# thomasjoergensen/RFAnalyzer

Measured on AMD Instinct MI355X. Metric: IQ Msamples/s + waterfall lines/s at 64k FFT; achieved HBM GB/s vs roofline, higher is better.
Workload: dtype f32; 1 GPU; config3: 65536-pt FFT, blackman window, s8 IQ, EMA + peak-hold, ring 500 rows, one stream per GPU; fft_size=65536, frames_per_call=500, input_format=s8, parallelism=streams1, avg=ema, ring_rows=500

## Files before the change

rfanalyzer_amd/csrc/engine.hip:

```cpp
#include <hip/hip_runtime.h>

#include <algorithm>
#include <cmath>
#include <cstdio>
#include <cstdlib>
#include <cstring>
#include <new>
#include <string>
#include <vector>

#include "../../include/rfa.h"
#include "fft_kernels.h"
#include "framer.h"

static constexpr size_t kStampWords = (size_t)2048 * 16 * 8;

using rfa::FftLaunch;

struct WinPlan {
    int count = 0;
    int block_bins = 0, n_jobs = 0, n_pieces = 0, n_folds = 0, n_slots = 0;
    void *d_plan = nullptr;
    size_t d_plan_cap = 0;
    float *d_out = nullptr;
// ... 893 lines not shown
    if (h->chan_on && h->have_tuning) {
        const float samples_per_hz = (float)n / (float)h->last_sample_rate;
        const int64_t f0 = h->last_frequency - h->last_sample_rate / 2;
        auto idx = [&](int64_t f) {
            const float x = (float)(f - f0) * samples_per_hz;
            const long long i = std::isnan(x) ? 0 : x >= 2147483647.0f ? 2147483647LL : x <= -2147483648.0f ? -2147483648LL
                                                                                                               : (long long)x;
            return (int)std::min<long long>(std::max<long long>(i, 0), n);
        };
        chan_first = idx(h->chan_start);
        chan_last = idx(h->chan_end);
    }
    const bool need_chan = chan_last > chan_first;
    h->chan_count = 0;
    h->chan_offset = 0;
    const bool need_win = h->win.count > 0;
    h->win.frames = h->win.offset = 0;
    float *state_rows = rows;
    bool rows_in_ring = false;
    if ((need_state || need_chan || need_win) && !rows) {
        if (h->d_ring && n_frames <= (size_t)h->ring_rows) {
            rows_in_ring = true;
        } else {
            int rc = ensure_device_buffer(h, (void **)&h->d_rows, &h->d_rows_cap, n_frames * (size_t)n * sizeof(float));
            if (rc) return rc;
            state_rows = h->d_rows;
        }
    }
    const bool flip = (long long)n_frames == (long long)h->ring_rows;
    const bool pipe = h->pipe_cus > 0 && need_state && rows_in_ring &&
                      (flip || (long long)n_frames + h->pipe_prev_frames <= (long long)h->ring_rows);
    if (!pipe) {
        int rc = join(h);
        if (rc) return rc;
    }
    const int par = (int)(h->pipe_k & 1);
    hipStream_t fft_stream = h->stream, state_stream = h->stream;
    if (pipe) {
        fft_stream = h->pipe_fft[h->logn > 17 ? 0 : par];
        state_stream = h->pipe_state;
        HIPCHK(h, hipEventRecord(h->pipe_in, h->stream));
        HIPCHK(h, hipStreamWaitEvent(fft_stream, h->pipe_in, 0));
        if (h->pipe_recorded[par]) HIPCHK(h, hipStreamWaitEvent(fft_stream, h->pipe_state_done[par], 0));
        if (flip) {
            std::swap(h->d_ring, h->d_ring_tmp);
            h->generation++;
        }
    }
    const bool raise_ok = h->d_peaks_st && h->d_state_part && rows_in_ring && !pipe &&
                          h->logn == 16 && (fmt == RFA_IN_S8 || fmt == RFA_IN_U8) && window == h->d_window &&
                          h->variant != 1 && h->diag == 0 && !h->d_stamps && (h->ring_logrs & rfa::kRingTile) &&
                          h->stage && (((uintptr_t)in | (uintptr_t)stride) & 15) == 0 &&
                          rfa::state_fused_plan(n, (int)n_frames, h->state_chunks, h->state_fused, nullptr, nullptr);
    const bool raise = raise_ok && h->shadow_fresh;
    FftLaunch a;
    a.in = (const uint8_t *)in;
    a.frame_stride = (long long)stride;
    a.n_frames = (int)n_frames;
    a.fmt = fmt;
    a.window = window;
    a.rows = state_rows;
    if (raise) a.peaks_st = h->d_peaks_st;
    if (pipe) a.cus = h->pipe_fft_cus;
    if (h->d_ring) {
        a.ring = h->d_ring;
        a.ring_rows = h->ring_rows;
        a.ring_base = h->write_index;
        a.ring_first = (int)std::max<long long>(0, (long long)n_frames - h->ring_rows);
        a.ring_logrs = h->ring_logrs;
    }
    int rc = launch_main(h, a, fft_stream);
    if (rc) return rc;
    if (pipe) {
        HIPCHK(h, hipEventRecord(h->pipe_fft_done[par], fft_stream));
        HIPCHK(h, hipStreamWaitEvent(state_stream, h->pipe_fft_done[par], 0));
    }
    if (need_state || need_chan || need_win) {
        rfa::StateLaunch s;
        s.n = n;
        s.n_frames = (int)n_frames;
        s.peaks = h->d_peaks;
        s.ema = h->d_ema;
        s.ema_alpha = h->cfg.ema_alpha;
        s.part = h->d_state_part;
        s.max_chunks = h->state_chunks;
        s.fused = h->state_fused;
        s.first_frame = (int)std::max<long long>(0, (long long)n_frames - rfa::ema_tail_frames(h->cfg.ema_alpha));
        s.peaks_st = raise_ok ? h->d_peaks_st : nullptr;
        s.raised = raise;
        s.stream = state_stream;
        if (rows_in_ring) {
            s.rows = h->d_ring;
            s.ring_rows = h->ring_rows;
            s.ring_base = h->write_index;
            s.ring_logrs = h->ring_logrs;
        } else {
            s.rows = state_rows;
            s.row_stride = n;
        }
        if (need_state) HIPCHK(h, rfa::launch_state(s));
        if (h->d_peaks) h->shadow_fresh = raise_ok;
        if (need_chan) {
            const int spans = rfa::channel_mean_spans(chan_last - chan_first);
            const size_t words = n_frames * (size_t)(spans > 1 ? 1 + spans : 1);
            if (pipe && words * sizeof(float) > h->d_chan_cap)
                HIPCHK(h, hipStreamSynchronize(state_stream));
            int rc = ensure_device_buffer(h, (void **)&h->d_chan, &h->d_chan_cap, words * sizeof(float));
            if (rc) return rc;
            HIPCHK(h, rfa::launch_channel_mean(s, chan_first, chan_last, h->d_chan,
                                               spans > 1 ? h->d_chan + n_frames : nullptr));
            h->chan_count = n_frames;
        }
        if (need_win) {
            rfa::WinLaunch w;
            w.rows = s.rows;
            w.row_stride = s.row_stride;
            w.ring_rows = s.ring_rows;
            w.ring_base = s.ring_base;
            w.ring_dir = -1;
            w.ring_logrs = s.ring_logrs;
            w.n_frames = (int)n_frames;
            w.stream = state_stream;
            int rc = run_windows(h, h->win, w, pipe ? state_stream : nullptr);
            if (rc) return rc;
        }
    }
    if (pipe) {
        HIPCHK(h, hipEventRecord(h->pipe_state_done[par], state_stream));
        h->pipe_recorded[par] = true;
        h->pipe_pending = true;
        h->pipe_prev_frames = (int)n_frames;
        h->pipe_k++;
    }
    if (h->d_ring) {
        const long long R = h->ring_rows;
        const long long last = (long long)n_frames - 1;
        for (long long f = std::max<long long>(0, (long long)n_frames - R); f < (long long)n_frames; f++)
            h->dirty[(size_t)((((long long)h->write_index - f) % R + R) % R)] = 1;
        h->read_index = (int)((((long long)h->write_index - last) % R + R) % R);
        h->write_index = h->read_index == 0 ? h->ring_rows - 1 : h->read_index - 1;
// ... 588 lines not shown
```

rfanalyzer_amd/csrc/fft_kernels.h:

```cpp
#pragma once

#include <hip/hip_runtime.h>
#include <stdint.h>

#include <vector>

namespace rfa {

constexpr int kRingTile = 0x100;
__host__ __device__ __forceinline__ int ring_lr(int code) { return code & 0xff; }
__host__ __device__ __forceinline__ int ring_logm(int code, int logn) { return logn - (code & 0xff); }
__host__ __device__ __forceinline__ int tile_pos(int i) {
    return (((i >> 6) & 15) << 11) | ((i >> 12) << 8) | ((i & 63) << 2) | ((i >> 10) & 3);
}
__host__ __device__ __forceinline__ int tile_sub(int p) {
    return ((((p >> 8) & 7) << 2 | (p & 3)) << 10) | ((p >> 11) << 6) | ((p >> 2) & 63);
}
constexpr int kRingTile2 = 0x200;
__host__ __device__ __forceinline__ int tile2_pos(int i) {
    const int k0 = i & 31, k1 = (i >> 5) & 31, tp = i >> 10;
    return ((k0 >> 1) << 11) | ((tp >> 2) << 8) | (((k0 & 1) | (k1 << 1)) << 2) | (tp & 3);
}
__host__ __device__ __forceinline__ int tile2_sub(int p) {
    const int w = p >> 11, j = (p >> 8) & 7, l = (p >> 2) & 63, e = p & 3;
    return ((l & 1) | (w << 1)) | ((l >> 1) << 5) | ((4 * j + e) << 10);
}
__host__ __device__ __forceinline__ int ring_pos(int t, int code, int logm) {
    const int lr = code & 0xff, sub = t >> lr;
    return ((t & ((1 << lr) - 1)) << logm) |
           ((code & kRingTile) ? tile_pos(sub) : (code & kRingTile2) ? tile2_pos(sub) : sub);
}
__host__ __device__ __forceinline__ int ring_bin(int p, int code, int logm) {
    const int lr = code & 0xff, q = p & ((1 << logm) - 1);
    return (((code & kRingTile) ? tile_sub(q) : (code & kRingTile2) ? tile2_sub(q) : q) << lr) | (p >> logm);
}

constexpr int kMaxLogM = 14;
constexpr int kMaxLogSplit = 3;

struct FftLaunch {
    const uint8_t *in = nullptr;
    long long frame_stride = 0;
    int n_frames = 0;
    int fmt = 0;
    int logn = 0;
    const float *window = nullptr;
    const float *window_il = nullptr;
    const float4 *window_cw = nullptr;
    const float2 *wide_tw = nullptr;
    const float2 *w64_tw = nullptr;
    const float2 *tw_coarse = nullptr;
    const float2 *tw_fine = nullptr;
    int tw_shift = 0;
    float *rows = nullptr;
    float *ring = nullptr;
    int ring_rows = 0;
    int ring_base = 0;
    int ring_first = 0;
    int ring_logrs = 0;
    float2 *complex_out = nullptr;
    float *peaks_st = nullptr;
    int dif_ss = 0;
    int stage = 1;
    int variant = 0;
    int diag = 0;
    unsigned long long *stamps = nullptr;
    int prio = 0;
    int phase_ticks = 0;
    int cus = 0;
    hipStream_t stream = nullptr;
};

hipError_t launch_fft(const FftLaunch &a);
bool wide_supported(int logn);
int ring_logrs_for(int logn, int fmt);
bool w64_format(int fmt);
constexpr int kWidePT = 32;
#ifndef RFA_RES16K
#define RFA_RES16K 0
#endif
inline int wide_logm(int logn) { return logn <= 14 ? logn : (RFA_RES16K && logn == 16 ? 14 : 15); }
std::vector<float2> wide_twiddles(int logn, int pt, int lm);
hipError_t launch_fft_wide(const FftLaunch &a);
std::vector<float2> w64_twiddles();
hipError_t launch_fft64(const FftLaunch &a);

struct DifLaunch {
    const uint8_t *in = nullptr;
    long long frame_stride = 0;
    int n_frames = 0;
    int fmt = 0;
    int logn = 0;
    const float *window = nullptr;
    const float2 *tw_c = nullptr;
    const float2 *tw_d = nullptr;
    const float2 *tw_cp = nullptr;
    const float2 *tw_dp = nullptr;
    float2 *z = nullptr;
    int pipe = 6;
    hipStream_t stream = nullptr;
};
constexpr int kDitLogM = 15;
constexpr int kMaxLogN = 20;
constexpr int kFmtDif = 5;
hipError_t launch_dif_front(const DifLaunch &a);
hipError_t launch_cols_to_rows(const float *cols, float *rows, int n_frames, int logn, hipStream_t st);
int dif_lo_points(bool pipe);
void dif_twiddles(int logn, int lo, std::vector<float2> &c, std::vector<float2> &d);

struct StateLaunch {
    const float *rows = nullptr;
    long long row_stride = 0;
    int ring_rows = 0;
    int ring_base = 0;
    int ring_logrs = 0;
    int n_frames = 0;
    int n = 0;
    float *peaks = nullptr;
    float *ema = nullptr;
    float ema_alpha = 0.f;
    float4 *part = nullptr;
    int max_chunks = 1;
    int fused = 1;
    int first_frame = 0;
    float *peaks_st = nullptr;
    bool raised = false;
    hipStream_t stream = nullptr;
};
hipError_t launch_state(const StateLaunch &a);
int ema_tail_frames(float alpha);
bool state_fused_plan(int n, int n_frames, int max_chunks, int fused, int *chunks, int *chunk_len);
int channel_mean_spans(int width);
hipError_t launch_channel_mean(const StateLaunch &a, int first, int last, float *out, float *partial);

struct DrawLaunch {
    const float *ring = nullptr;
    const float *peaks = nullptr;
    int ring_rows = 0, n = 0, read_index = 0;
    int ring_logrs = 0;
    int width = 0, fft_height = 0, avg_length = 0;
    int start = 0, first_pixel = 0, last_pixel = 0;
    float samples_per_px = 0.f, min_db = 0.f, db_width = 0.f, scale = 0.f;
    const unsigned *colormap = nullptr;
    int colormap_size = 0;
    unsigned *colors = nullptr;
    const int2 *rows = nullptr;
    int n_rows = 0;
    float *avg_rows = nullptr;
    float *path_y = nullptr;
    float *peaks_y = nullptr;
    float *autoscale = nullptr;
    hipStream_t stream = nullptr;
};
hipError_t launch_draw(const DrawLaunch &a);
hipError_t launch_row_windows(const float *row, int ring_logrs, int n, const int *lo, const int *hi, int count,
                              float *peak, float *avg, hipStream_t s);

struct WinLaunch {
    const float *rows = nullptr;
    long long row_stride = 0;
    int ring_rows = 0, ring_base = 0, ring_dir = -1;
    int ring_logrs = 0;
    int n = 0, n_frames = 0;
    int n_windows = 0;
    int block_bins = 0;
    const int4 *jobs = nullptr;
    int n_jobs = 0;
    const int4 *pieces = nullptr;
    const int4 *folds = nullptr;
    int n_folds = 0, n_slots = 0;
    float *peak = nullptr, *avg = nullptr;
    double *psum = nullptr;
    float *pmax = nullptr;
    hipStream_t stream = nullptr;
};
constexpr int kWinNarrow = 32;
constexpr int kWinWave = 1024;
inline int win_piece_bins(int n) { return n < 4096 ? n : 4096; }
inline int win_block_bins(int n, int ring_code) {
    return (ring_code & (kRingTile | kRingTile2)) ? 4096 << ring_lr(ring_code) : win_piece_bins(n);
}
hipError_t launch_batch_windows(const WinLaunch &a);

hipError_t launch_fill(float *p, long long count, float value, hipStream_t s);
// ... 12 lines not shown
```

rfanalyzer_amd/csrc/fft_kernels.hip:

```cpp
#include <hip/hip_runtime.h>
#include <math.h>

#include <algorithm>
#include <cstdlib>
#include <type_traits>

#include "fft_common.h"
#include "fft_kernels.h"
#include "wave.h"

namespace rfa {
template <int LOGM>
struct Geo {
    static constexpr int M = 1 << LOGM;
    static constexpr int TPF = M / 16;
    static constexpr int SLOTS = TPF >= 256 ? 1 : 256 / TPF;
    static constexpr int THREADS = TPF * SLOTS;
    static constexpr int PADM = M + M / 8;
    static constexpr int NP16 = LOGM / 4;
    static constexpr int LASTR = 1 << (LOGM % 4);
    static constexpr int NPASS = NP16 + (LASTR > 1 ? 1 : 0);
};

__device__ __forceinline__ int pad(int e) { return e + ((e >> 4) << 1); }
// ... 439 lines not shown
        const float4 x4 = *reinterpret_cast<const float4 *>(state_row(a, f) + bin);
        const float xs[4] = {x4.x, x4.y, x4.z, x4.w};
#pragma unroll
        for (int k = 0; k < 4; k++) state_step(pk[k], nan[k], emi[k], b[k], xs[k], al);
        am *= keep;
    }
    float4 *out = a.part + (size_t)c * a.n + bin;
#pragma unroll
    for (int k = 0; k < 4; k++) out[k] = state_summary(pk[k], nan[k], am, b[k], emi[k]);
}

__global__ void state_combine_kernel(StateLaunch a, int chunks) {
    const int pos = blockIdx.x * blockDim.x + threadIdx.x;
    if (pos >= a.n) return;
    const int lr = state_logrs(a), bin = ring_bin(pos, lr, ring_logm(lr, ilog2_dev(a.n)));
    float pk = a.peaks ? a.peaks[bin] : 0.f;
    float em = a.ema ? a.ema[bin] : 0.f;
    for (int c = 0; c < chunks; c++) {
        const float4 p = a.part[(size_t)c * a.n + pos];
        pk = peak_max(pk, p.x);
        em = (!state_finite(em) || p.y < 0.0f) ? p.w : fmaf(p.y, em, p.z);
    }
    if (a.peaks) a.peaks[bin] = pk;
    if (a.ema) a.ema[bin] = em;
}

#ifndef RFA_STATE_BUF
#define RFA_STATE_BUF 1
#endif
#ifndef RFA_STATE_UNROLL
#define RFA_STATE_UNROLL 4
#endif
#ifndef RFA_STATE_LOAD_AUX
#define RFA_STATE_LOAD_AUX 0
#endif
template <int CH, bool RAISED = false>
__global__ void __launch_bounds__(256) state_fused_kernel(StateLaunch a, int chunk_len) {
    constexpr int TPC = 256 / CH, BPB = 4 * TPC;
    __shared__ float4 part[CH][BPB];
    const int c = threadIdx.x / TPC, l = threadIdx.x % TPC;
    const int bin = blockIdx.x * BPB + 4 * l;
    const int tail = a.n_frames - a.first_frame;
    {
        const int f0 = a.first_frame + c * chunk_len, f1 = min(a.n_frames, f0 + chunk_len);
        const float al = a.ema_alpha, keep = 1.0f - al;
        float pk[4], emi[4], b[4];
        bool nan[4];
#pragma unroll
        for (int k = 0; k < 4; k++) pk[k] = emi[k] = -INFINITY, b[k] = 0.0f, nan[k] = false;
        float am = 1.0f;
        auto step = [&](float4 x4) {
            const float xs[4] = {x4.x, x4.y, x4.z, x4.w};
#pragma unroll
            for (int k = 0; k < 4; k++) {
                if constexpr (RAISED) {
                    emi[k] = ema_step(emi[k], xs[k], al);
                    b[k] = fmaf(al, xs[k] - b[k], b[k]);
                } else {
                    state_step(pk[k], nan[k], emi[k], b[k], xs[k], al);
                }
            }
            am *= keep;
        };
        auto peak_step = [&](float4 x4) {
            const float xs[4] = {x4.x, x4.y, x4.z, x4.w};
#pragma unroll
            for (int k = 0; k < 4; k++) pk[k] = fmaxf(pk[k], xs[k]), nan[k] |= xs[k] != xs[k];
        };
        auto frames = [&](int fa, int fb, auto &&each) {
            if (RFA_STATE_BUF && a.ring_rows > 0 && (long long)a.ring_rows * a.n * 4 < (1ll << 31)) {
                const unsigned rowb = (unsigned)a.n * 4u;
                const rsrc_t rs = make_rsrc(a.rows, (unsigned)a.ring_rows * rowb);
                int rr = (a.ring_base - fa) % a.ring_rows;
                if (rr < 0) rr += a.ring_rows;
#pragma unroll RFA_STATE_UNROLL
                for (int f = fa; f < fb; f++) {
                    each(__builtin_bit_cast(float4, __builtin_amdgcn_raw_buffer_load_b128(rs, (int)((unsigned)rr * rowb + (unsigned)bin * 4u), 0, RFA_STATE_LOAD_AUX)));
                    rr = rr == 0 ? a.ring_rows - 1 : rr - 1;
                }
            } else {
#pragma unroll 4
                for (int f = fa; f < fb; f++) each(*reinterpret_cast<const float4 *>(state_row(a, f) + bin));
            }
        };
        if constexpr (!RAISED) {
            if (a.first_frame > 0 && a.peaks) {
                const int plen = (a.first_frame + CH - 1) / CH;
                frames(min(a.first_frame, c * plen), min(a.first_frame, (c + 1) * plen), peak_step);
            }
        }
        frames(f0, f1, step);
#pragma unroll
        for (int k = 0; k < 4; k++) part[c][4 * l + k] = state_summary(pk[k], nan[k], am, b[k], emi[k]);
    }
    __syncthreads();
    const int lr = state_logrs(a), lm = ring_logm(lr, ilog2_dev(a.n));
    const bool full = (CH - 1) * chunk_len < tail;
    for (int i = threadIdx.x; i < BPB; i += 256) {
        const int pos = blockIdx.x * BPB + i, gb = ring_bin(pos, lr, lm);
        float p = a.peaks ? a.peaks[gb] : 0.f;
        float em = a.ema ? a.ema[gb] : 0.f;
        if constexpr (RAISED) p = peak_max(p, a.peaks_st[pos]);
        auto fold = [&](auto all) {
#pragma unroll
            for (int cc = 0; cc < CH; cc++) {
                const bool any = decltype(all)::value || cc * chunk_len < tail;
                const float4 q = part[cc][i];
                if constexpr (!RAISED) p = peak_max(p, q.x);
                em = !any ? em : (!state_finite(em) || q.y < 0.0f) ? q.w : fmaf(q.y, em, q.z);
            }
        };
        if (full) fold(std::true_type{});
        else fold(std::false_type{});
        if (a.peaks) a.peaks[gb] = p;
        if (a.peaks && a.peaks_st) a.peaks_st[pos] = p;
        if (a.ema) a.ema[gb] = em;
    }
}

#ifdef RFA_AB_BUILD
static const bool kStateTileOff = std::getenv("RFA_STATE_TILE") && std::atoi(std::getenv("RFA_STATE_TILE")) == 0;
#else
static constexpr bool kStateTileOff = false;
#endif

bool state_fused_plan(int n, int n_frames, int max_chunks, int fused, int *chunks, int *chunk_len) {
    const int c = std::min(max_chunks, (n_frames + 7) / 8);
    if (c < 8 || !fused) return false;
    const int ch = c >= 32 ? 32 : c >= 16 ? 16 : 8;
    if (n % (1024 / ch)) return false;
    if (chunks) *chunks = ch;
    if (chunk_len) *chunk_len = (n_frames + ch - 1) / ch;
    return true;
}

int ema_tail_frames(float alpha) {
    const double keep = 1.0 - (double)alpha, bound = std::ldexp(1.0, -51);
    if (!(keep > 0.0)) return 1;
    if (!(keep < 1.0)) return 0x7fffffff;
    const double t0 = std::ceil(std::log(bound) / std::log(keep));
    if (!(t0 < 1.0e9)) return 0x7fffffff;
    int t = std::max(1, (int)t0);
    while (t > 1 && std::pow(keep, t - 1) <= bound) t--;
    while (std::pow(keep, t) > bound) t++;
    return t;
}

hipError_t launch_state(const StateLaunch &a) {
    if (a.n_frames <= 0) return hipSuccess;
    const int tpb = 256;
    if (a.raised && !(a.peaks && a.peaks_st && state_fused_plan(a.n, a.n_frames, a.max_chunks, a.fused, nullptr, nullptr) &&
                      a.part && (a.ring_logrs & kRingTile)))
        return hipErrorInvalidValue;
    if (a.ring_rows > 0 && !(a.ring_logrs & kRingTile) && a.ring_logrs >= 3 && a.ring_logrs <= 5 && !kStateTileOff) {
        const int m = a.n >> a.ring_logrs;
        if (m % 64 == 0) {
            auto k = a.ring_logrs == 5 ? state_tile_kernel<5> : a.ring_logrs == 4 ? state_tile_kernel<4>
                                                                                  : state_tile_kernel<3>;
            hipLaunchKernelGGL(k, dim3(m / 64, (1 << a.ring_logrs) / 8), dim3(256), 0, a.stream, a);
            return hipGetLastError();
        }
    }
    const int bx = (a.n + tpb - 1) / tpb;
    int chunks = a.part ? std::min(a.max_chunks, (a.n_frames + 7) / 8) : 1;
    int ch = 0, len = 0;
    if (a.part && state_fused_plan(a.n, a.n_frames, a.max_chunks, a.fused, &ch, &len)) {
        StateLaunch b = a;
        b.first_frame = !a.ema ? (a.raised ? a.n_frames : 0) : std::min(std::max(a.first_frame, 0), a.n_frames);
        if (b.first_frame > 0) {
            const int tail = a.n_frames - b.first_frame;
            if (!state_fused_plan(a.n, tail, a.max_chunks, a.fused, &ch, &len)) {
                if (a.n % 128 == 0) ch = 8, len = std::max(1, (tail + 7) / 8);
                else b.first_frame = 0;
            }
        }
        auto k = a.raised ? (ch == 32 ? state_fused_kernel<32, true> : ch == 16 ? state_fused_kernel<16, true>
                                                                                 : state_fused_kernel<8, true>)
                          : (ch == 32 ? state_fused_kernel<32> : ch == 16 ? state_fused_kernel<16> : state_fused_kernel<8>);
        hipLaunchKernelGGL(k, dim3(a.n / (1024 / ch)), dim3(256), 0, a.stream, b, len);
        return hipGetLastError();
    }
    if (chunks > 1) {
        const int len = (a.n_frames + chunks - 1) / chunks;
        chunks = (a.n_frames + len - 1) / len;
        hipLaunchKernelGGL(state_partial_kernel, dim3((a.n / 4 + tpb - 1) / tpb, chunks), dim3(tpb), 0, a.stream, a,
                           len);
        hipLaunchKernelGGL(state_combine_kernel, dim3(bx), dim3(tpb), 0, a.stream, a, chunks);
    } else {
        hipLaunchKernelGGL(state_kernel, dim3(bx), dim3(tpb), 0, a.stream, a);
    }
    return hipGetLastError();
}

__global__ void __launch_bounds__(256) channel_mean_kernel(StateLaunch a, int first, int last, int span, float *out,
                                                          float *partial) {
    __shared__ float part[4];
    const int f = blockIdx.x, t = threadIdx.x;
    const float *row = state_row(a, f);
    const int lr = state_logrs(a), lm = ring_logm(lr, ilog2_dev(a.n));
    const int lo = first + blockIdx.y * span, hi = min(last, lo + span);
    float s = 0.0f;
    int i = lo + t;
    for (; i + 3 * 256 < hi; i += 4 * 256) {
        const float x0 = row[ring_pos(i, lr, lm)], x1 = row[ring_pos(i + 256, lr, lm)];
        const float x2 = row[ring_pos(i + 512, lr, lm)], x3 = row[ring_pos(i + 768, lr, lm)];
        s = (((s + x0) + x1) + x2) + x3;
    }
    for (; i < hi; i += 256) s += row[ring_pos(i, lr, lm)];
    s = wave_reduce(s, [](float x, float y) { return x + y; });
    if ((t & 63) == 0) part[t >> 6] = s;
    __syncthreads();
    if (t == 0) {
        const float sum = ((part[0] + part[1]) + part[2]) + part[3];
        if (gridDim.y == 1) out[f] = sum / (float)(last - first);
        else partial[(size_t)f * gridDim.y + blockIdx.y] = sum;
    }
}

__global__ void channel_mean_fold_kernel(int n_frames, int spans, int width, const float *partial, float *out) {
    const int f = blockIdx.x * blockDim.x + threadIdx.x;
    if (f >= n_frames) return;
    float s = 0.0f;
    for (int k = 0; k < spans; k++) s += partial[(size_t)f * spans + k];
    out[f] = s / (float)width;
}

int channel_mean_spans(int width) { return std::min(64, std::max(1, (width + 16383) / 16384)); }

// ... 115 lines not shown
```

rfanalyzer_amd/csrc/fft_wide.hip:

```cpp
#include <hip/hip_runtime.h>

#include <algorithm>
#include <cstdlib>
#include <cmath>
#include <type_traits>
#include <vector>

#include "fft_common.h"
#include "fft_kernels.h"
#include "fft_w8.h"

namespace rfa {

[[maybe_unused]] constexpr int kSc1 = 16;
#ifndef RFA_RING_SC1
#define RFA_RING_SC1 1
#endif
#ifndef RFA_WIN_UPFRONT
#define RFA_WIN_UPFRONT 16
#endif
#ifndef RFA_RES_HOIST
#define RFA_RES_HOIST 1
#endif
#ifndef RFA_STG_OWNQ
#define RFA_STG_OWNQ 1
#endif
#ifndef RFA_STG_OWN
#define RFA_STG_OWN 1
#endif
#ifndef RFA_PKR_WIN_UPFRONT
#define RFA_PKR_WIN_UPFRONT 4
#endif
#ifndef RFA_WIDE_KR1
#define RFA_WIDE_KR1 0
#endif
template <int LOGM, int PT>
struct WGeo {
    static constexpr int M = 1 << LOGM;
    static constexpr int TPF = M / PT;
    static constexpr int THREADS = TPF < 256 ? 256 : TPF;
    static constexpr int SLOTS = THREADS / TPF;
    static constexpr int HALF = (RFA_WIDE_KR1 && LOGM == 13) ? M : M / 2;
    static constexpr int HALFP = HALF + HALF / 32;
    static constexpr int R1 = LOGM >= 14 ? 32 : 16;
    static constexpr int R2 = M / (32 * R1);
    static constexpr int P1_ROW = R1 - 1;
    static constexpr int TW_P1 = 32 * P1_ROW;
    static constexpr int LO = TPF > 256 ? 32 : 16;
    static constexpr int P2_ROW = R2 - 1;
    static constexpr bool A_ALIAS = LOGM == 13 && R1 == 16 && R2 == 16 && LO == 16 && TPF / LO <= 32;
    static constexpr int TW_P2A = A_ALIAS ? 0 : (TPF / LO) * P2_ROW;
    static constexpr int TW_P2B = LO * P2_ROW;
    static_assert(!A_ALIAS || (32 * R1 * LO == M && P1_ROW == R2 - 1), "A rows = pass-1 rows");
    static constexpr int TW_LDS = TW_P1 + TW_P2A + TW_P2B;
    static constexpr int LDS_BYTES = (TW_LDS + SLOTS * HALFP) * 8;
};

template <int Q, int LOGM, int PT>
struct WPass {
    using G = WGeo<LOGM, PT>;
    static constexpr int R = Q == 0 ? 32 : (Q == 1 ? G::R1 : G::R2);
    static constexpr int P = Q == 0 ? 1 : (Q == 1 ? 32 : 32 * G::R1);
    static constexpr int NB = PT / R;
    static constexpr int STRIDE = G::M / R;
};

__device__ __forceinline__ constexpr int padw(int e) { return e + (e >> 5); }

template <typename T>
__device__ __forceinline__ float2 tw_ld(const T *p) { return lds_ld2(p); }

template <int Q, int LOGM, int PT, int KR = 2, bool XST = false>
__device__ __forceinline__ void exchange(float2 (&v)[PT], float2 *buf, int tid) {
    using G = WGeo<LOGM, PT>;
    using W = WPass<Q, LOGM, PT>;
    using N = WPass<Q + 1, LOGM, PT>;
    static_assert(N::R >= KR && (W::NB == 1 || W::NB % KR == 0), "round split needs radix >= KR");
    constexpr int PART = G::M / KR, PARTP = PART + PART / 32;
    float2 in[KR][PT / KR];
    const int wk = tid & (W::P - 1);
    const int wbase = padw((tid - wk) * W::R + wk);
    const int rbase = padw(tid);
    const int my_part = tid / (G::TPF / KR);
#pragma unroll
// ... 463 lines not shown
    static_assert(!OWN || (PT == 32 && G::TPF == M / 32), "OWN: one pre-stage sample per thread per M/32");
    auto stage_half = [&](int f, int half) {
        if constexpr (OWN)
            stage_half_own<HALF_BYTES, G::THREADS, BPS, M / 32>(
                a.in + (size_t)f * (size_t)a.frame_stride + (half ? HALF_BYTES : 0), half ? buf : buf + QP);
        else if constexpr (SPLIT)
            stage_frame<HALF_BYTES, G::THREADS>(a.in + (size_t)f * (size_t)a.frame_stride + (half ? HALF_BYTES : 0),
                                                half ? buf : buf + QP);
    };
    if constexpr (STG) {
        const int f0 = frame_of(u0);
        if (u0 < items && f0 < a.n_frames) {
            if constexpr (SPLIT) {
                stage_half(f0, 0);
                stage_half(f0, 1);
            } else if constexpr (QST) {
                stage_q(f0);
            } else if constexpr (QSTB) {
                stage_qb(u0);
            } else {
                stage_frame<M * RS * BPS, G::THREADS>(a.in + (size_t)f0 * (size_t)a.frame_stride, buf);
            }
        }
    }

#ifdef RFA_AB_BUILD
    if (STG && a.phase_ticks > 0 && blockIdx.x >= gridDim.x / 2) {
        const unsigned long long t0 = __builtin_amdgcn_s_memrealtime();
        while (__builtin_amdgcn_s_memrealtime() - t0 < (unsigned long long)a.phase_ticks) __builtin_amdgcn_s_sleep(2);
    }
#endif
    int it_count = 0;
    auto stamp = [&](int u, int k) {
        if constexpr ((DIAG & 32) != 0) {
            const int it = it_count;
            if (threadIdx.x == 0 && it < 16)
                a.stamps[((size_t)blockIdx.x * 16 + it) * 8 + k] = __builtin_amdgcn_s_memrealtime();
        }
    };
    int pending_st = 0;

    static_assert(!PKR || (SPLIT && DIAG == 0 && PT == 32), "peak raise: the staged 64 K 8-bit kernel");
    typedef float pk4v __attribute__((ext_vector_type(4)));
    auto raise_peak = [&](float *dst, float x) {
        const int bits = __builtin_bit_cast(int, x);
        if (bits >= 0)
            (void)__hip_atomic_fetch_max(reinterpret_cast<int *>(dst), bits, __ATOMIC_RELAXED, __HIP_MEMORY_SCOPE_AGENT);
        else
            (void)__hip_atomic_fetch_min(reinterpret_cast<unsigned *>(dst), (unsigned)bits, __ATOMIC_RELAXED,
                                         __HIP_MEMORY_SCOPE_AGENT);
    };

#if RFA_RES_HOIST
    auto body = [&]<int RF>(int u, int unext) {
#else
    auto body = [&](int u, int unext) {
#endif
        stamp(u, 0);
        int tid = tid0;
        asm volatile("" : "+v"(tid));
        int z;
        asm volatile("s_mov_b32 %0, 0" : "=s"(z));
        const float2 *tp1 = twp1 + z, *tp2 = twp2 + z;
        int frame, r;
        int dif_r = 0;
        if constexpr (RS == 1) {
            frame = u * G::SLOTS + slot;
            r = 0;
            if constexpr (dif) {
                frame = u / a.dif_ss;
                dif_r = u - frame * a.dif_ss;
            }
        } else {
            const int g = u / (8 * RS), rem = u - g * (8 * RS);
            r = rem >> 3;
            frame = g * 8 + (rem & 7);
        }
        const bool active = frame < a.n_frames;
        constexpr int SB0 = FMT == 4 ? 4 : BPS;
        const rsrc_t in_rs =
            make_rsrc(a.in + (size_t)(active ? frame : 0) * (size_t)a.frame_stride + (size_t)dif_r * (M * 8),
                      active ? (unsigned)(n * BPS) : 0u);
        const int planar_im = n * 4;

        float2 v[PT];
        using RawT = typename Raw<FMT>::T;
        const RawT *lraw = reinterpret_cast<const RawT *>(SPLIT ? buf + QP : buf);
        if constexpr (STG) {
            const int younger = pending_st;
            if constexpr (OWN || OWNQ) {
                if (younger >= 63) asm volatile("s_waitcnt vmcnt(63)" ::: "memory");
                else if (younger >= 32) asm volatile("s_waitcnt vmcnt(32)" ::: "memory");
                else asm volatile("s_waitcnt vmcnt(0)" ::: "memory");
            } else {
                if (younger >= 63) asm volatile("s_waitcnt vmcnt(63) lgkmcnt(0)\n\ts_barrier" ::: "memory");
                else if (younger >= 32) asm volatile("s_waitcnt vmcnt(32) lgkmcnt(0)\n\ts_barrier" ::: "memory");
                else asm volatile("s_waitcnt vmcnt(0) lgkmcnt(0)\n\ts_barrier" ::: "memory");
            }
            stamp(u, 1);
        }
        if constexpr (RS == 1) {
            const rsrc_t w_rs = make_rsrc(a.window, dif ? 0 : n * 4);
            constexpr int SB = SB0;
            typename Raw<FMT>::T raw[PT];
    #pragma unroll
            for (int idx = 0; idx < PT; idx++) {
                const int so = G::TPF * (idx >> 5) + (M / 32) * (idx & 31);
                if constexpr (DIAG & 1) raw[idx] = synth_raw<FMT>(so + tid);
                else if constexpr (STG) {
                    if (QSTB && idx >= PT / 2) raw[idx] = buf_load_raw<FMT>(in_rs, tid * SB, so * SB, planar_im);
                    else raw[idx] = lraw[so + tid];
                } else raw[idx] = buf_load_raw<FMT>(in_rs, tid * SB, so * SB, planar_im);
            }
    #pragma unroll
            for (int idx = 0; idx < PT; idx++) {
                const int so = G::TPF * (idx >> 5) + (M / 32) * (idx & 31);
                const float w = ((DIAG & 16) || dif) ? 1.0f : buf_load_f32(w_rs, tid * 4, so * 4);
                const float2 x = convert_raw<FMT>(raw[idx]);
                v[idx] = make_float2(x.x * w, x.y * w);
            }
        } else {
            const int planar = planar_im;
            [&]<int... Rs>(std::integer_sequence<int, Rs...>) {
#if RFA_RES_HOIST
                (((RF >= 0 ? RF == Rs : r == Rs) ? prestage<LOGM, PT, RS, FMT, Rs, STG, (DIAG & 16) != 0, QST ? QN : JS,
#else
                ((r == Rs ? prestage<LOGM, PT, RS, FMT, Rs, STG, (DIAG & 16) != 0, QST ? QN : JS,
#endif
                                     RS == 2 && Rs == 1 && FMT <= 2 && (DIAG & 16) == 0, QCH,
                                     PKR ? RFA_PKR_WIN_UPFRONT : RFA_WIN_UPFRONT>(
                                v, a.window_il, a.wide_tw, in_rs, tid, planar, lraw, a.window_cw)
                          : void()), ...);
            }(std::make_integer_sequence<int, RS>{});
        }

    #pragma unroll
        for (int b = 0; b < PT / 32; b++)
            if constexpr (!(DIAG & 4)) dftw<32, W8>(&v[b * 32]);
        stamp(u, 2);
        if constexpr (STG) {
            lds_barrier();
            stamp(u, 7);
            if constexpr (SPLIT) {
                const int fn = frame_of(unext);
                if (unext < items && fn < a.n_frames) stage_half(fn, 0);
            }
        }
        if constexpr (!(DIAG & 8)) exchange<0, LOGM, PT, KR, STG>(v, buf, tid);
        stamp(u, 3);
        if constexpr (!(DIAG & 4)) pass1<LOGM, PT, W8>(v, tid, tp1);
        if constexpr (!(DIAG & 8)) exchange<1, LOGM, PT, KR, STG>(v, buf, tid);
        stamp(u, 4);
        if constexpr (STG) {
            const int fn = frame_of(unext);
            if (unext < items && fn < a.n_frames) {
                if constexpr (SPLIT) stage_half(fn, 1);
                else if constexpr (QST) stage_q(fn);
                else if constexpr (QSTB) stage_qb(unext);
                else stage_frame<M * RS * BPS, G::THREADS>(a.in + (size_t)fn * (size_t)a.frame_stride, buf);
            }
        }
        if constexpr (!(DIAG & 4)) pass2<LOGM, PT, W8>(v, tid, tp2);
        stamp(u, 5);
        if constexpr ((DIAG & 12) != 0) {
    #pragma unroll
            for (int q = 0; q < PT; q++) asm volatile("" : "+v"(v[q].x), "+v"(v[q].y));
        }

        if (!active) return;
        if constexpr (PKR) {
            constexpr float db_off = -kDbPerLog2 * (float)(2 * (LOGM + 1));
            int rr = (a.ring_base - frame) % a.ring_rows;
            if (rr < 0) rr += a.ring_rows;
            const int tp = (tid >> 6) * 2048 + (tid & 63) * 4;
            float *blk = a.peaks_st + (size_t)r * M;
            const rsrc_t p_rs = make_rsrc(blk, M * 4);
            const rsrc_t ring_rs = make_rsrc(a.ring + (size_t)rr * n + (size_t)r * M, M * 4);
            pk4v shadow[PT / 4];
#pragma unroll
            for (int j = 0; j < PT / 4; j++)
                shadow[j] = __builtin_bit_cast(pk4v, __builtin_amdgcn_raw_buffer_load_b128(p_rs, tp * 4, j * 1024, 0));
            __builtin_amdgcn_sched_barrier(0);
            float d[PT];
#pragma unroll
            for (int j = 0; j < PT / 4; j++) {
#pragma unroll
                for (int e = 0; e < 4; e++) d[4 * j + e] = db_unscaled(v[(4 * j + e + 16) & 31], db_off);
                if constexpr (RFA_RING_SC1) buf_store_f32x4(d[4 * j], d[4 * j + 1], d[4 * j + 2], d[4 * j + 3], ring_rs, tp * 4, j * 1024);
                else buf_store_f32x4_wb(d[4 * j], d[4 * j + 1], d[4 * j + 2], d[4 * j + 3], ring_rs, tp * 4, j * 1024);
            }
            __builtin_amdgcn_sched_barrier(0);
#pragma unroll
            for (int j = 0; j < PT / 4; j++) {
                const pk4v sh = shadow[j];
                if (d[4 * j] > sh.x || d[4 * j + 1] > sh.y || d[4 * j + 2] > sh.z || d[4 * j + 3] > sh.w) {
#pragma unroll
                    for (int e = 0; e < 4; e++)
                        if (d[4 * j + e] > sh[e]) raise_peak(blk + tp + j * 256 + e, d[4 * j + e]);
                }
            }
            pending_st = PT / 4;
            stamp(u, 6);
            return;
        }
        const int ors = dif ? a.dif_ss : RS, orr = dif ? dif_r : r;
        const int on = dif ? M * a.dif_ss : n;
        if constexpr (COMPLEX_OUT) {
            const rsrc_t o_rs = make_rsrc(a.complex_out + (size_t)frame * on, on * 8);
    #pragma unroll
            for (int b = 0; b < PT / G::R2; b++)
    #pragma unroll
                for (int t = 0; t < G::R2; t++)
                    buf_store_f32x2(v[b * G::R2 + t], o_rs, (ors * tid + orr) * 8,
                                    ors * (G::TPF * b + t * (M / G::R2)) * 8);
        } else {
            constexpr float db_off_c = -kDbPerLog2 * (float)(2 * (LOGM + (RS == 1 ? 0 : RS == 2 ? 1 : RS == 4 ? 2 : 3)));
            const float db_off = dif ? db_offset(LOGM + (31 - __builtin_clz(a.dif_ss))) : db_off_c;
            const bool to_ring = a.ring && frame >= a.ring_first;
            int rr = 0;
            if (to_ring) {
                rr = (a.ring_base - frame) % a.ring_rows;
                if (rr < 0) rr += a.ring_rows;
            }
            const bool rm = (RS > 1 || dif) && a.ring_logrs > 0;
            constexpr bool TILE_OK = LOGM == 15 && PT == 32 && G::TPF == 1024 && !dif;
            const bool tile = TILE_OK && (a.ring_logrs & kRingTile) != 0;
            const rsrc_t row_rs = make_rsrc(a.rows ? a.rows + (size_t)frame * on + (dif ? (size_t)orr * M : 0) : nullptr,
                                            a.rows ? (dif ? M : on) * 4 : 0);
            const rsrc_t ring_rs = make_rsrc(to_ring ? a.ring + (size_t)rr * on + ((rm || tile) ? (size_t)orr * M : 0) : nullptr,
                                             to_ring ? ((rm || tile) ? M : on) * 4 : 0);
// ... 52 lines not shown
                            }(),
                            ...);
                    }(std::make_integer_sequence<int, PT>{});
                    return;
                }
    #pragma unroll
                for (int b = 0; b < PT / G::R2; b++) {
    #pragma unroll
                    for (int t = 0; t < G::R2; t++) {
                        const float2 x = v[b * G::R2 + t];
                        const float db = db_unscaled(x, db_off);
                        const int so = ((ors * (G::TPF * b + t * (M / G::R2)) + on / 2) & (on - 1)) * 4;
                        const int so_rm = ((G::TPF * b + t * (M / G::R2) + M / 2) & (M - 1)) * 4;
                        if constexpr (DIAG & 2) {
                            asm volatile("" ::"v"(db));
                        } else {
                            if constexpr (decltype(nat_c)::value) {
                                if constexpr (dif) buf_store_f32(db, row_rs, tid * 4, so_rm);
                                else buf_store_f32(db, row_rs, vo, so);
                            }
                            if constexpr (decltype(ring_c)::value) {
                                if constexpr (decltype(rm_c)::value) buf_store_f32(db, ring_rs, tid * 4, so_rm);
                                else buf_store_f32(db, ring_rs, vo, so);
                            }
                        }
                    }
                }
            };
            using T_ = std::true_type;
            using F_ = std::false_type;
            pending_st = (DIAG & 2) ? 0 : (a.rows ? PT : 0) + (to_ring ? PT : 0);
            if (a.rows && to_ring) {
                if constexpr (RS > 1 || dif) {
                    if (rm) epilogue(T_{}, T_{}, T_{});
                    else epilogue(T_{}, T_{}, F_{});
                } else {
                    epilogue(T_{}, T_{}, F_{});
                }
            } else if (a.rows) {
                epilogue(T_{}, F_{}, F_{});
            } else if (to_ring) {
                if constexpr (RS > 1 || dif) {
                    if (rm) epilogue(F_{}, T_{}, T_{});
                    else epilogue(F_{}, T_{}, F_{});
                } else {
                    epilogue(F_{}, T_{}, F_{});
                }
            }
            stamp(u, 6);
        }
    };
#if RFA_RES_HOIST
    auto loop = [&]<int RF>() {
        for (int u = u0; u < items; it_count++) {
            const int un = next_item(u);
            body.template operator()<RF>(u, un);
            u = un;
        }
    };
    if constexpr (RS == 2 && !dif) {
        if (gridDim.x % (8 * RS) == 0) {
            if (((u0 % (8 * RS)) >> 3) == 0) loop.template operator()<0>();
            else loop.template operator()<1>();
        } else {
            loop.template operator()<-1>();
        }
    } else {
        loop.template operator()<-1>();
    }
#else
    for (int u = u0; u < items; it_count++) {
        const int un = next_item(u);
        body(u, un);
        u = un;
    }
#endif
}

template <int LOGM, int PT, int RS, int FMT, bool CO, int DIAG = 0, bool STG = false, bool PKR = false>
static hipError_t launch_wide_one(const FftLaunch &a) {
    using G = WGeo<LOGM, PT>;
    auto kern = &fft_wide_kernel<LOGM, PT, RS, FMT, CO, DIAG, STG, PKR>;
    if (a.peaks_st && !(PKR && a.ring && (a.ring_logrs & kRingTile) && !a.rows && a.ring_first == 0 &&
                        a.n_frames <= a.ring_rows))
        return hipErrorInvalidValue;
    const size_t lds = (size_t)G::LDS_BYTES;
    if (!a.wide_tw) return hipErrorInvalidValue;
    if (RS == 2 && FMT <= 2 && (DIAG & 16) == 0 && !a.window_cw) return hipErrorInvalidValue;
    static bool attr = false;
    if (!attr) {
        hipError_t e = hipFuncSetAttribute(reinterpret_cast<const void *>(kern),
                                           hipFuncAttributeMaxDynamicSharedMemorySize, (int)lds);
        if (e != hipSuccess) return e;
        attr = true;
    }
    const int work = FMT == kFmtDif ? a.n_frames * a.dif_ss : a.n_frames;
    const int items = RS == 1 ? (work + G::SLOTS - 1) / G::SLOTS : ((a.n_frames + 7) / 8) * 8 * RS;
    if (items <= 0) return hipSuccess;
    int blocks = items;
    if (STG) {
        static int cus = 0, occ = 0;
        if (!cus) {
            int dev = 0;
            (void)hipGetDevice(&dev);
            if (hipDeviceGetAttribute(&cus, hipDeviceAttributeMultiprocessorCount, dev) != hipSuccess) cus = 256;
            if (hipOccupancyMaxActiveBlocksPerMultiprocessor(&occ, reinterpret_cast<const void *>(kern), G::THREADS,
                                                             lds) != hipSuccess || occ < 1)
                occ = 1;
        }
        blocks = std::min(items, (a.cus > 0 ? a.cus : cus) * occ);
#ifdef RFA_AB_BUILD
        if (const char *g = std::getenv("RFA_WIDE_GRID")) blocks = std::min(blocks, std::max(16, std::atoi(g)));
#endif
    }
    hipLaunchKernelGGL(kern, dim3(blocks), dim3(G::THREADS), lds, a.stream, a);
    return hipGetLastError();
}

int ring_logrs_for(int logn, int fmt) {
    if (logn > 17 && logn <= kMaxLogN) return logn - kDitLogM;
    if (!wide_supported(logn) || logn <= 14) return 0;
    if (logn == 16 && w64_format(fmt)) return 1 | kRingTile2;
    return (logn - wide_logm(logn)) | kRingTile;
}

template <int LOGM, int PT, int RS, bool CO>
static hipError_t wide_by_fmt(const FftLaunch &a) {
    if constexpr (CO) {
        return a.fmt == 3 ? launch_wide_one<LOGM, PT, RS, 3, true>(a) : hipErrorInvalidValue;
    } else {
        using G = WGeo<LOGM, PT>;
        constexpr int M = 1 << LOGM;
        const bool stg = a.stage && ((reinterpret_cast<uintptr_t>(a.in) | (uintptr_t)a.frame_stride) & 15) == 0;
        constexpr bool stg8 = G::SLOTS == 1 && M * RS * 2 <= G::HALFP * 8;
        constexpr bool stg16 = G::SLOTS == 1 && M * RS * 4 <= G::HALFP * 8;
        if constexpr (stg8 && LOGM == 15 && RS == 2) {
            if (stg && a.peaks_st && a.fmt == 0) return launch_wide_one<LOGM, PT, RS, 0, false, 0, true, true>(a);
// ... 130 lines not shown
```

Before: 340,800 Msamples/s.

## Split peak-raise at EMA tail so FFT skips shadow compare on tail frames

The FFT epilogue's peak-hold raise (load shadow peaks, compare, update) now only runs for frames before the EMA tail start. Tail frames just write dB rows to the ring, and the state kernel processes those tail frames with full state_step, including the peak update. The split point is computed once by a shared state_split helper. This trims shadow loads and compares from the FFT kernel, but the state kernel does somewhat more work on the tail, and an optional compile flag adds a two-body loop variant.

```diff
diff --git a/rfanalyzer_amd/csrc/engine.hip b/rfanalyzer_amd/csrc/engine.hip
--- a/rfanalyzer_amd/csrc/engine.hip
+++ b/rfanalyzer_amd/csrc/engine.hip
@@ -969,7 +969,10 @@
                           h->variant != 1 && h->diag == 0 && !h->d_stamps && (h->ring_logrs & rfa::kRingTile) &&
                           h->stage && (((uintptr_t)in | (uintptr_t)stride) & 15) == 0 &&
                           rfa::state_fused_plan(n, (int)n_frames, h->state_chunks, h->state_fused, nullptr, nullptr);
-    const bool raise = raise_ok && h->shadow_fresh;
+    bool raise = raise_ok && h->shadow_fresh;
+    const int first_frame = rfa::state_split(n, (int)n_frames, h->state_chunks, h->state_fused, h->d_ema != nullptr,
+                                             h->cfg.ema_alpha, raise, nullptr, nullptr);
+    raise = raise && first_frame > 0;
     FftLaunch a;
     a.in = (const uint8_t *)in;
     a.frame_stride = (long long)stride;
@@ -977,7 +980,7 @@
     a.fmt = fmt;
     a.window = window;
     a.rows = state_rows;
-    if (raise) a.peaks_st = h->d_peaks_st;
+    if (raise) a.peaks_st = h->d_peaks_st, a.raise_below = first_frame;
     if (pipe) a.cus = h->pipe_fft_cus;
     if (h->d_ring) {
         a.ring = h->d_ring;
@@ -1002,7 +1005,7 @@
         s.part = h->d_state_part;
         s.max_chunks = h->state_chunks;
         s.fused = h->state_fused;
-        s.first_frame = (int)std::max<long long>(0, (long long)n_frames - rfa::ema_tail_frames(h->cfg.ema_alpha));
+        s.first_frame = first_frame;
         s.peaks_st = raise_ok ? h->d_peaks_st : nullptr;
         s.raised = raise;
         s.stream = state_stream;
diff --git a/rfanalyzer_amd/csrc/fft_kernels.h b/rfanalyzer_amd/csrc/fft_kernels.h
--- a/rfanalyzer_amd/csrc/fft_kernels.h
+++ b/rfanalyzer_amd/csrc/fft_kernels.h
@@ -60,6 +60,7 @@
     int ring_logrs = 0;
     float2 *complex_out = nullptr;
     float *peaks_st = nullptr;
+    int raise_below = 0;
     int dif_ss = 0;
     int stage = 1;
     int variant = 0;
@@ -130,6 +131,8 @@
 hipError_t launch_state(const StateLaunch &a);
 int ema_tail_frames(float alpha);
 bool state_fused_plan(int n, int n_frames, int max_chunks, int fused, int *chunks, int *chunk_len);
+int state_split(int n, int n_frames, int max_chunks, int fused, bool ema, float alpha, bool raised, int *chunks,
+                int *chunk_len);
 int channel_mean_spans(int width);
 hipError_t launch_channel_mean(const StateLaunch &a, int first, int last, float *out, float *partial);
 
diff --git a/rfanalyzer_amd/csrc/fft_kernels.hip b/rfanalyzer_amd/csrc/fft_kernels.hip
--- a/rfanalyzer_amd/csrc/fft_kernels.hip
+++ b/rfanalyzer_amd/csrc/fft_kernels.hip
@@ -515,14 +515,7 @@
         auto step = [&](float4 x4) {
             const float xs[4] = {x4.x, x4.y, x4.z, x4.w};
 #pragma unroll
-            for (int k = 0; k < 4; k++) {
-                if constexpr (RAISED) {
-                    emi[k] = ema_step(emi[k], xs[k], al);
-                    b[k] = fmaf(al, xs[k] - b[k], b[k]);
-                } else {
-                    state_step(pk[k], nan[k], emi[k], b[k], xs[k], al);
-                }
-            }
+            for (int k = 0; k < 4; k++) state_step(pk[k], nan[k], emi[k], b[k], xs[k], al);
             am *= keep;
         };
         auto peak_step = [&](float4 x4) {
@@ -569,7 +562,7 @@
             for (int cc = 0; cc < CH; cc++) {
                 const bool any = decltype(all)::value || cc * chunk_len < tail;
                 const float4 q = part[cc][i];
-                if constexpr (!RAISED) p = peak_max(p, q.x);
+                p = peak_max(p, q.x);
                 em = !any ? em : (!state_finite(em) || q.y < 0.0f) ? q.w : fmaf(q.y, em, q.z);
             }
         };
@@ -609,11 +602,31 @@
     return t;
 }
 
+int state_split(int n, int n_frames, int max_chunks, int fused, bool ema, float alpha, bool raised, int *chunks,
+                int *chunk_len) {
+    int ch = 0, len = 0;
+    if (!state_fused_plan(n, n_frames, max_chunks, fused, &ch, &len)) return 0;
+    int first = !ema ? (raised ? n_frames : 0) : std::max(0, n_frames - std::min(n_frames, ema_tail_frames(alpha)));
+    if (first > 0) {
+        const int tail = n_frames - first;
+        if (!state_fused_plan(n, tail, max_chunks, fused, &ch, &len)) {
+            if (n % 128 == 0) ch = 8, len = std::max(1, (tail + 7) / 8);
+            else first = 0;
+        }
+    }
+    if (chunks) *chunks = ch;
+    if (chunk_len) *chunk_len = len;
+    return first;
+}
+
 hipError_t launch_state(const StateLaunch &a) {
     if (a.n_frames <= 0) return hipSuccess;
     const int tpb = 256;
     if (a.raised && !(a.peaks && a.peaks_st && state_fused_plan(a.n, a.n_frames, a.max_chunks, a.fused, nullptr, nullptr) &&
-                      a.part && (a.ring_logrs & kRingTile)))
+                      a.part && (a.ring_logrs & kRingTile) &&
+                      a.first_frame == state_split(a.n, a.n_frames, a.max_chunks, a.fused, a.ema != nullptr, a.ema_alpha,
+                                                   true, nullptr, nullptr) &&
+                      a.first_frame > 0))
         return hipErrorInvalidValue;
     if (a.ring_rows > 0 && !(a.ring_logrs & kRingTile) && a.ring_logrs >= 3 && a.ring_logrs <= 5 && !kStateTileOff) {
         const int m = a.n >> a.ring_logrs;
@@ -629,14 +642,7 @@
     int ch = 0, len = 0;
     if (a.part && state_fused_plan(a.n, a.n_frames, a.max_chunks, a.fused, &ch, &len)) {
         StateLaunch b = a;
-        b.first_frame = !a.ema ? (a.raised ? a.n_frames : 0) : std::min(std::max(a.first_frame, 0), a.n_frames);
-        if (b.first_frame > 0) {
-            const int tail = a.n_frames - b.first_frame;
-            if (!state_fused_plan(a.n, tail, a.max_chunks, a.fused, &ch, &len)) {
-                if (a.n % 128 == 0) ch = 8, len = std::max(1, (tail + 7) / 8);
-                else b.first_frame = 0;
-            }
-        }
+        b.first_frame = state_split(a.n, a.n_frames, a.max_chunks, a.fused, a.ema != nullptr, a.ema_alpha, a.raised, &ch, &len);
         auto k = a.raised ? (ch == 32 ? state_fused_kernel<32, true> : ch == 16 ? state_fused_kernel<16, true>
                                                                                  : state_fused_kernel<8, true>)
                           : (ch == 32 ? state_fused_kernel<32> : ch == 16 ? state_fused_kernel<16> : state_fused_kernel<8>);
diff --git a/rfanalyzer_amd/csrc/fft_wide.hip b/rfanalyzer_amd/csrc/fft_wide.hip
--- a/rfanalyzer_amd/csrc/fft_wide.hip
+++ b/rfanalyzer_amd/csrc/fft_wide.hip
@@ -30,6 +30,9 @@
 #endif
 #ifndef RFA_PKR_WIN_UPFRONT
 #define RFA_PKR_WIN_UPFRONT 4
+#endif
+#ifndef RFA_PKR_TWO_BODIES
+#define RFA_PKR_TWO_BODIES 0
 #endif
 #ifndef RFA_WIDE_KR1
 #define RFA_WIDE_KR1 0
@@ -599,8 +602,10 @@
     };
 
 #if RFA_RES_HOIST
-    auto body = [&]<int RF>(int u, int unext) {
+    auto body = [&]<int RF, bool RZ = PKR>(int u, int unext) {
 #else
+    constexpr bool RZ = PKR;
+    constexpr int RF = -1;
     auto body = [&](int u, int unext) {
 #endif
         stamp(u, 0);
@@ -675,7 +680,7 @@
                 ((r == Rs ? prestage<LOGM, PT, RS, FMT, Rs, STG, (DIAG & 16) != 0, QST ? QN : JS,
 #endif
                                      RS == 2 && Rs == 1 && FMT <= 2 && (DIAG & 16) == 0, QCH,
-                                     PKR ? RFA_PKR_WIN_UPFRONT : RFA_WIN_UPFRONT>(
+                                     RZ ? RFA_PKR_WIN_UPFRONT : RFA_WIN_UPFRONT>(
                                 v, a.window_il, a.wide_tw, in_rs, tid, planar, lraw, a.window_cw)
                           : void()), ...);
             }(std::make_integer_sequence<int, RS>{});
@@ -715,7 +720,7 @@
         }
 
         if (!active) return;
-        if constexpr (PKR) {
+        if constexpr (RZ) {
             constexpr float db_off = -kDbPerLog2 * (float)(2 * (LOGM + 1));
             int rr = (a.ring_base - frame) % a.ring_rows;
             if (rr < 0) rr += a.ring_rows;
@@ -723,6 +728,19 @@
             float *blk = a.peaks_st + (size_t)r * M;
             const rsrc_t p_rs = make_rsrc(blk, M * 4);
             const rsrc_t ring_rs = make_rsrc(a.ring + (size_t)rr * n + (size_t)r * M, M * 4);
+            if (!(RFA_PKR_TWO_BODIES && RF >= 0) && frame >= a.raise_below) {
+#pragma unroll
+                for (int j = 0; j < PT / 4; j++) {
+                    float d[4];
+#pragma unroll
+                    for (int e = 0; e < 4; e++) d[e] = db_unscaled(v[(4 * j + e + 16) & 31], db_off);
+                    if constexpr (RFA_RING_SC1) buf_store_f32x4(d[0], d[1], d[2], d[3], ring_rs, tp * 4, j * 1024);
+                    else buf_store_f32x4_wb(d[0], d[1], d[2], d[3], ring_rs, tp * 4, j * 1024);
+                }
+                pending_st = PT / 4;
+                stamp(u, 6);
+                return;
+            }
             pk4v shadow[PT / 4];
 #pragma unroll
             for (int j = 0; j < PT / 4; j++)
@@ -881,7 +899,21 @@
     };
 #if RFA_RES_HOIST
     auto loop = [&]<int RF>() {
-        for (int u = u0; u < items; it_count++) {
+        int u = u0;
+        if constexpr (PKR && RFA_PKR_TWO_BODIES && RF >= 0) {
+            for (; u < items && frame_of(u) < a.raise_below; it_count++) {
+                const int un = next_item(u);
+                body.template operator()<RF, true>(u, un);
+                u = un;
+            }
+            for (; u < items; it_count++) {
+                const int un = next_item(u);
+                body.template operator()<RF, false>(u, un);
+                u = un;
+            }
+            return;
+        }
+        for (; u < items; it_count++) {
             const int un = next_item(u);
             body.template operator()<RF>(u, un);
             u = un;
@@ -911,7 +943,7 @@
     using G = WGeo<LOGM, PT>;
     auto kern = &fft_wide_kernel<LOGM, PT, RS, FMT, CO, DIAG, STG, PKR>;
     if (a.peaks_st && !(PKR && a.ring && (a.ring_logrs & kRingTile) && !a.rows && a.ring_first == 0 &&
-                        a.n_frames <= a.ring_rows))
+                        a.n_frames <= a.ring_rows && a.raise_below > 0 && a.raise_below <= a.n_frames))
         return hipErrorInvalidValue;
     const size_t lds = (size_t)G::LDS_BYTES;
     if (!a.wide_tw) return hipErrorInvalidValue;
```

After: 346,400 Msamples/s (median of 6 runs). 1.02x the previous value.
